# emanuele-artioli/elvis

Hardware: AMD Instinct MI355X
Metric: restored 1080p frames/sec, SinSR 4x path (ELVIS v2 Downsample) (higher is better)
Workload: dtype f16; 1 GPU; 30-frame 1920x1080 synthetic clip per GPU, ELVIS v2 Downsample (SinSR 4x), block 8, levels 0-3, weights seed 0 (random init), quantize=True; frames_per_gpu=30, parallelism=single GPU, gn_fused_into_conv=True, frames_per_invocation=15

## Files before the change

elvis_amd/_build.py:

```python
from __future__ import annotations

import os
import shutil
import subprocess
import sys
from concurrent.futures import ThreadPoolExecutor

HERE = os.path.dirname(os.path.abspath(__file__))
CSRC = os.path.join(HERE, "csrc")
LIBDIR = os.path.join(HERE, "lib")
OBJDIR = os.path.join(LIBDIR, "obj")
LIBPATH = os.path.join(LIBDIR, "libelvis_amd.so")
SOURCES = ["conv.hip", "conv_f32.hip", "dcn.hip", "swin.hip", "api.hip", "glue.hip", "misc.hip", "norm.hip", "attn.hip", "degrade.hip", "presley_degrade.hip", "classical.hip", "shrink.hip", "quality.hip", "handoff.hip"]
ARCH = "gfx950"
FLAGS = ["-O3", "-std=c++17", "-fPIC", f"--offload-arch={ARCH}", "-Wno-unused-result",
         "-ffp-contract=off"]
EXTRA_FLAGS = {"dcn.hip": ["-mllvm", "-pragma-unroll-threshold=262144"]}


def _hipcc() -> str:
    for cand in (shutil.which("hipcc"), "/opt/rocm/bin/hipcc"):
        if cand and os.path.exists(cand):
            return cand
    raise RuntimeError("hipcc not found; libelvis_amd cannot be built")


def _stale(target: str, deps) -> bool:
    if not os.path.exists(target):
        return True
    t = os.path.getmtime(target)
    return any(os.path.getmtime(d) > t for d in deps)


def build(force: bool = False, verbose: bool = True) -> str:
    os.makedirs(OBJDIR, exist_ok=True)
    hipcc = _hipcc()
    headers = [os.path.join(CSRC, f) for f in os.listdir(CSRC) if f.endswith((".h", ".inc"))]
    headers.append(os.path.join(os.path.dirname(HERE), "include", "elvis_amd.h"))
    jobs = []
    for src in SOURCES:
        s = os.path.join(CSRC, src)
        o = os.path.join(OBJDIR, src.replace(".hip", ".o"))
        if force or _stale(o, [s] + headers):
            jobs.append((s, o))

    def compile_one(job):
# ... 25 lines not shown
```

elvis_amd/_lib.py:

```python
from __future__ import annotations

import ctypes as C
import os
import threading
from typing import Optional

HERE = os.path.dirname(os.path.abspath(__file__))
LIBPATH = os.environ.get("ELVIS_AMD_LIB") or os.path.join(HERE, "lib", "libelvis_amd.so")

F32, F16 = 0, 1
ROUND_CV2, ROUND_HALF_UP = 0, 1
SSIM_LUMA, SSIM_CHANNELS = 0, 1
SSIM_REFLECT, SSIM_VALID = 0, 1
SSIM_PAD_AUTO = -1

_lock = threading.Lock()
_lib: Optional[C.CDLL] = None

vp, i32, f32, i64, f64 = C.c_void_p, C.c_int, C.c_float, C.c_longlong, C.c_double


class ConvDesc(C.Structure):
    _fields_ = [(n, C.c_int) for n in (
        "dtype", "n", "h", "w", "cin", "cin_pitch", "cin2", "cin2_pitch", "cout", "cout_pitch",
# ... 11 lines not shown
    "elvis_tile_accumulate_f32": [vp, vp, vp, vp, vp, vp, i32, i32, i32, i32, i32, i32, i32, f32, vp],
    "elvis_tile_normalize_u8": [vp, vp, vp, i32, i32, i32, vp],
    "elvis_sse_u8": [vp, vp, vp, vp, vp, i32, i32, i32, i32, vp],
    "elvis_block_ssim_u8": [vp, vp, vp, vp, i32, i32, i32, i32, i32, vp],
    "elvis_mask_bbox_u8": [vp, vp, i32, i32, i32, vp],
    "elvis_apply_mask_u8": [vp, vp, vp, i32, i32, i32, i32, i32, vp],
    "elvis_ssim_workspace_bytes": [i32, i32, i32, i32],
    "elvis_ssim_mean_f64": [vp, vp, vp, vp, vp, vp, vp, i32, i32, i32, i32, i32, i32, f64, f64, f64, i32, f64, vp],
    "elvis_u8_to_float": [vp, vp, i32, i32, i32, i32, i32, f32, f32, i32, i32, vp],
    "elvis_float_to_u8": [vp, i32, vp, vp, i32, i32, i32, i32, f32, f32, i32, i32, vp],
    "elvis_conv_packed_weight_bytes": [C.POINTER(ConvDesc)],
    "elvis_conv_pack_weights": [C.POINTER(ConvDesc), vp, vp, vp],
    "elvis_conv2d": [C.POINTER(ConvDesc), vp, vp, vp, vp, vp, i32, vp, vp, vp, vp, vp],
    "elvis_conv_stats_tiles": [C.POINTER(ConvDesc)],
    "elvis_conv_kernel_name": [C.POINTER(ConvDesc), C.c_char_p, C.c_size_t],
    "elvis_conv_kernel_name_for_call": [C.POINTER(ConvDesc), i32, i32, C.c_char_p, C.c_size_t],
    "elvis_conv_x3_eligible": [C.POINTER(ConvDesc)],
    "elvis_conv_debug_set": [C.c_char_p, i32],
    "elvis_gn_partials_to_sums": [vp, i32, i32, i32, vp, i32, i32, vp],
    "elvis_groupnorm_workspace_floats": [i32, i32, i32, i32],
    "elvis_groupnorm_sums": [vp, i32, i32, i32, i32, i32, vp, i32, i32, vp, vp],
    "elvis_groupnorm_affine": [vp, vp, vp, vp, vp, vp, vp, i32, i32, i32, i32, f32, vp],
    "elvis_affine_act": [vp, vp, i32, i32, i32, i32, i32, i32, vp, vp, i32, vp],
    "elvis_layernorm": [vp, vp, i32, i64, i32, i32, i32, vp, vp, f32, vp],
    "elvis_swin_packed_bytes": [i32, i32, i32],
    "elvis_swin_pack_weights": [vp, vp, vp, i32, i32, i32, vp],
    "elvis_swin_mlp": [vp, vp, vp, vp, vp, vp, vp, i64, i32, i32, i32, i32, f32, vp],
    "elvis_swin_ln_linear": [vp, vp, vp, vp, vp, vp, i64, i32, i32, i32, i32, f32, vp],
    "elvis_swin_pack_proj_mlp": [vp, vp, vp, vp, i32, i32, vp],
    "elvis_swin_proj_mlp": [vp, vp, vp, vp, vp, vp, vp, vp, vp, i64, i32, i32, i32, i32, i32, f32, vp],
    "elvis_window_attention": [vp, vp, i32, i32, i32, i32, i32, i32, i32, i32, i32, i32, vp, f32, vp],
    "elvis_bicubic_upsample": [vp, vp, i32, i32, i32, i32, i32, i32, i32, i32, vp],
    "elvis_vq_nearest": [vp, vp, vp, i32, i64, i32, i32, i32, vp, i32, vp],
    "elvis_pad_reflect_axpy": [vp, vp, i32, i32, i32, i32, i32, i32, i32, i32, i32, i32, f32, vp, f32, vp],
    "elvis_crop_copy": [vp, vp, i32, i32, i32, i32, i32, i32, i32, i32, i32, vp],
    "elvis_convert_act": [vp, i32, vp, i32, i64, i32, vp],
    "elvis_degrade_downsample_u8": [vp, vp, vp, i32, i32, i32, i32, i32, i32, i32, vp],
    "elvis_degrade_gaussian_u8": [vp, vp, vp, i32, i32, i32, i32, i32, i32, i32, f32, f32, f32, vp],
    "elvis_degrade_dct_u8": [vp, vp, vp, vp, vp, i32, i32, i32, i32, i32, i32, i32, vp],
    "elvis_degrade_scale_u8": [vp, vp, vp, i32, i32, i32, i32, i32, i32, i32, vp, vp, vp, i32, vp],
    "elvis_degrade_gaussian_fx_u8": [vp, vp, vp, i32, i32, i32, i32, i32, i32, i32, i32, i32, i32, vp],
    "elvis_rgb_to_i420_u8": [vp, vp, i32, i32, i32, i32, vp],
    "elvis_classical_lanczos_u8": [vp, vp, vp, i32, i32, i32, i32, i32, i32, i32, vp, vp],
    "elvis_classical_unsharp_u8": [vp, vp, vp, i32, i32, i32, i32, i32, i32, i32, i32, vp, vp, i32, vp],
    "elvis_temporal_blend_u8": [vp, vp, i32, i64, f64, f64, vp],
    "elvis_block_gather_u8": [vp, vp, vp, vp, i32, i32, i32, i32, i32, i32, i32, i32, i32, vp],
    "elvis_shrink_select_topk": [vp, vp, vp, i32, i32, i32, i32, vp],
    "elvis_shrink_passes_plan": [i32, i32, i32, i32, vp, vp, vp, i32],
    "elvis_shrink_select_passes": [vp, vp, vp, vp, vp, vp, i32, i32, i32, i32, i32, i32, i32, vp],
    "elvis_stretch_index": [vp, vp, i32, i32, i32, i32, i32, i32, vp],
    "elvis_dcnv2": [vp, vp, vp, vp, vp, i32, i32, i32, i32, i32, i32, i32, i32, i32, i32, i32, i32, vp],
    "elvis_temporal_stack": [vp, vp, i32, i32, i32, i32, i32, i32, i32, i32, vp],
    "elvis_plane_merge": [vp, vp, vp, i32, i32, i32, i32, i32, i32, vp],
}


def lib() -> C.CDLL:
    global _lib
    if _lib is not None:
        return _lib
    with _lock:
        if _lib is not None:
            return _lib
        if not os.path.exists(LIBPATH):
            raise RuntimeError(
                f"libelvis_amd.so not found at {LIBPATH}. Build it with `python -m elvis_amd._build` "
# ... 67 lines not shown
```

elvis_amd/csrc/norm.hip:

```cpp
#include "common.h"

namespace {

template <typename T> struct Vec16 {
    uint4 raw;
    __device__ __forceinline__ float get(int i) const { return to_f(reinterpret_cast<const T*>(&raw)[i]); }
    __device__ __forceinline__ void set(int i, float v) { reinterpret_cast<T*>(&raw)[i] = from_f<T>(v); }
};

template <typename T>
__global__ __launch_bounds__(256) void gn_channel_sums_kernel(const T* __restrict__ x, int hw, int c, int pitch,
                                                              int px_per_block, float* __restrict__ partials) {
    constexpr int VEC = DT<T>::VEC;
    extern __shared__ float red[];
    const int cv = (c + VEC - 1) / VEC;
    const int pl_count = 256 / cv;
    const int tid = threadIdx.x;
    const int vec = tid % cv, plane = tid / cv;
    const int n = blockIdx.y;
    const long long p0 = (long long)blockIdx.x * px_per_block;
    long long p1 = p0 + px_per_block;
    if (p1 > hw) p1 = hw;
    float s[VEC], ss[VEC];
#pragma unroll
// ... 32 lines not shown
    }
}

__global__ __launch_bounds__(256) void gn_partials_reduce_kernel(const float* __restrict__ partials,
                                                                 int tiles_per_image, int c,
                                                                 double* __restrict__ sums, int ctot, int coff) {
    __shared__ double ra[256], rb[256];
    const int ch = blockIdx.x, n = blockIdx.y, tid = threadIdx.x;
    double a = 0, b = 0;
    const float* base = partials + ((long long)n * tiles_per_image * c + ch) * 2;
    for (int t = tid; t < tiles_per_image; t += 256) {
        a += (double)base[(long long)t * c * 2 + 0];
        b += (double)base[(long long)t * c * 2 + 1];
    }
    ra[tid] = a;
    rb[tid] = b;
    __syncthreads();
    for (int o = 128; o > 0; o >>= 1) {
        if (tid < o) {
            ra[tid] += ra[tid + o];
            rb[tid] += rb[tid + o];
        }
        __syncthreads();
    }
    if (tid == 0) {
        sums[((long long)n * ctot + coff + ch) * 2 + 0] = ra[0];
        sums[((long long)n * ctot + coff + ch) * 2 + 1] = rb[0];
    }
}

__global__ __launch_bounds__(256) void gn_partials_reduce4_kernel(const float* __restrict__ partials,
                                                                  int tiles_per_image, int c,
                                                                  double* __restrict__ sums, int ctot, int coff) {
    __shared__ double red[8][256];
    const int ch = blockIdx.x * 4, n = blockIdx.y, tid = threadIdx.x;
    double acc[8] = {0, 0, 0, 0, 0, 0, 0, 0};
    const float* base = partials + ((long long)n * tiles_per_image * c + ch) * 2;
    for (int t = tid; t < tiles_per_image; t += 256) {
        const float4* p4 = reinterpret_cast<const float4*>(base + (long long)t * c * 2);
        const float4 u = p4[0], v = p4[1];
        acc[0] += (double)u.x; acc[1] += (double)u.y; acc[2] += (double)u.z; acc[3] += (double)u.w;
        acc[4] += (double)v.x; acc[5] += (double)v.y; acc[6] += (double)v.z; acc[7] += (double)v.w;
    }
#pragma unroll
    for (int k = 0; k < 8; ++k) red[k][tid] = acc[k];
    __syncthreads();
    for (int o = 128; o > 0; o >>= 1) {
        if (tid < o) {
#pragma unroll
            for (int k = 0; k < 8; ++k) red[k][tid] += red[k][tid + o];
        }
        __syncthreads();
    }
    if (tid < 8) sums[((long long)n * ctot + coff + ch) * 2 + tid] = red[tid][0];
}

__global__ void gn_affine_kernel(const double* __restrict__ sums, const float* __restrict__ gamma,
                                 const float* __restrict__ beta, const float* __restrict__ scale,
                                 const float* __restrict__ shift, float* __restrict__ pa, float* __restrict__ pb,
                                 int n, int hw, int c, int groups, float eps) {
    int i = blockIdx.x * blockDim.x + threadIdx.x;
    if (i >= n * c) return;
    int ni = i / c, ch = i - ni * c;
    int cpg = c / groups;
    int g = ch / cpg;
    double s = 0, ss = 0;
    for (int k = 0; k < cpg; ++k) {
        s += sums[((long long)ni * c + g * cpg + k) * 2 + 0];
        ss += sums[((long long)ni * c + g * cpg + k) * 2 + 1];
    }
    double cnt = (double)hw * cpg;
    double mean = s / cnt;
    double var = ss / cnt - mean * mean;
    if (var < 0) var = 0;
    float rstd = (float)(1.0 / sqrt(var + (double)eps));
    float ga = gamma ? gamma[ch] : 1.f, be = beta ? beta[ch] : 0.f;
    float a = rstd * ga;
    float b = be - (float)mean * a;
    if (scale) {
        float sc = 1.f + scale[ch];
        a *= sc;
        b = b * sc + (shift ? shift[ch] : 0.f);
    } else if (shift) {
        b += shift[ch];
    }
    pa[i] = a;
    pb[i] = b;
// ... 97 lines not shown
    ELVIS_REQUIRE(n > 0 && hw > 0 && c > 0 && pitch >= c && pitch % 8 == 0, "elvis_groupnorm_sums: bad shape c=%d pitch=%d", c, pitch);
    int vec = dtype == ELVIS_F16 ? 8 : 4;
    int cv = (c + vec - 1) / vec;
    ELVIS_REQUIRE(cv <= 256, "elvis_groupnorm_sums: too many channels (%d)", c);
    ELVIS_REQUIRE(sums_coff >= 0 && sums_coff + c <= sums_ctot, "elvis_groupnorm_sums: channel slice [%d,%d) outside %d", sums_coff, sums_coff + c, sums_ctot);
    ELVIS_REQUIRE((uintptr_t)x % 16 == 0, "elvis_groupnorm_sums: x must be 16-byte aligned");
    int pl = 256 / cv;
    int px_per_block = 0;
    int gx = gn_blocks(dtype, hw, c, &px_per_block);
    size_t lds = (size_t)pl * c * 2 * sizeof(float);
    ELVIS_REQUIRE(lds <= 64 * 1024, "elvis_groupnorm_sums: LDS budget exceeded");
    if (dtype == ELVIS_F16)
        hipLaunchKernelGGL(gn_channel_sums_kernel<half_t>, dim3(gx, n), dim3(256), lds, (hipStream_t)stream,
                           (const half_t*)x, hw, c, pitch, px_per_block, workspace);
    else if (dtype == ELVIS_F32)
        hipLaunchKernelGGL(gn_channel_sums_kernel<float>, dim3(gx, n), dim3(256), lds, (hipStream_t)stream,
                           (const float*)x, hw, c, pitch, px_per_block, workspace);
    else
        ELVIS_REQUIRE(false, "elvis_groupnorm_sums: bad dtype");
    ELVIS_CHECK_LAUNCH("elvis_groupnorm_sums");
    elvis_note_launch(dtype == ELVIS_F16 ? "gn_channel_sums_kernel<half>" : "gn_channel_sums_kernel<float>");
    hipLaunchKernelGGL(gn_partials_reduce_kernel, dim3(c, n), dim3(256), 0, (hipStream_t)stream, workspace, gx, c, sums,
                       sums_ctot, sums_coff);
    ELVIS_CHECK_LAUNCH("elvis_groupnorm_sums(reduce)");
    return ELVIS_OK;
}

extern "C" int elvis_gn_partials_to_sums(const float* partials, int tiles_per_image, int n, int c, double* sums,
                                         int sums_ctot, int sums_coff, elvis_stream_t stream) {
    ELVIS_REQUIRE(partials && sums && tiles_per_image > 0 && n > 0 && c > 0, "elvis_gn_partials_to_sums: bad argument");
    ELVIS_REQUIRE(sums_coff >= 0 && sums_coff + c <= sums_ctot, "elvis_gn_partials_to_sums: channel slice outside buffer");
    const bool four = c % 4 == 0 && ((uintptr_t)partials & 15) == 0;
    if (four)
        hipLaunchKernelGGL(gn_partials_reduce4_kernel, dim3(c / 4, n), dim3(256), 0, (hipStream_t)stream, partials,
                           tiles_per_image, c, sums, sums_ctot, sums_coff);
    else
        hipLaunchKernelGGL(gn_partials_reduce_kernel, dim3(c, n), dim3(256), 0, (hipStream_t)stream, partials,
                           tiles_per_image, c, sums, sums_ctot, sums_coff);
    ELVIS_CHECK_LAUNCH("elvis_gn_partials_to_sums");
    elvis_note_launch(four ? "gn_partials_reduce4_kernel" : "gn_partials_reduce_kernel");
    return ELVIS_OK;
}

extern "C" int elvis_groupnorm_affine(const double* sums, const float* gamma, const float* beta, const float* scale,
                                      const float* shift, float* pa, float* pb, int n, int hw, int c, int groups,
                                      float eps, elvis_stream_t stream) {
    ELVIS_REQUIRE(sums && pa && pb, "elvis_groupnorm_affine: null pointer");
    ELVIS_REQUIRE(n > 0 && hw > 0 && c > 0 && groups > 0 && c % groups == 0, "elvis_groupnorm_affine: c=%d not divisible by groups=%d", c, groups);
    int total = n * c;
    hipLaunchKernelGGL(gn_affine_kernel, dim3((total + 255) / 256), dim3(256), 0, (hipStream_t)stream, sums, gamma,
                       beta, scale, shift, pa, pb, n, hw, c, groups, eps);
    ELVIS_CHECK_LAUNCH("elvis_groupnorm_affine");
    elvis_note_launch("gn_affine_kernel");
    return ELVIS_OK;
}

extern "C" int elvis_affine_act(const void* x, void* y, int dtype, int n, int hw, int c, int pitch_in, int pitch_out,
                                const float* pa, const float* pb, int act, elvis_stream_t stream) {
    ELVIS_REQUIRE(x && y && pa && pb, "elvis_affine_act: null pointer");
    ELVIS_REQUIRE(n > 0 && hw > 0 && c > 0 && pitch_in >= c && pitch_out >= c && pitch_in % 8 == 0 && pitch_out % 8 == 0,
                  "elvis_affine_act: bad shape");
    ELVIS_REQUIRE(act == 0 || act == 2, "elvis_affine_act: act must be 0 or 2");
    ELVIS_REQUIRE(((uintptr_t)x | (uintptr_t)y) % 16 == 0, "elvis_affine_act: x and y must be 16-byte aligned");
    int vec = dtype == ELVIS_F16 ? 8 : 4;
    long long total_vec = (long long)n * hw * ((c + 7) / 8 * (8 / vec));
    int grid = (int)((total_vec + 255) / 256);
    if (grid > 256 * 32) grid = 256 * 32;
// ... 40 lines not shown
```

elvis_amd/ops.py:

```python
from __future__ import annotations

import ctypes as C
from dataclasses import dataclass
from typing import Optional

import numpy as np
import torch

from . import _lib as L
from ._lib import ConvDesc, check, lib, ptr


def _s(t: torch.Tensor) -> int:
    return torch.cuda.current_stream(t.device).cuda_stream


def pitch_for(c: int) -> int:
    return (c + 7) // 8 * 8


@dataclass
class Act:
    t: torch.Tensor
    c: int
# ... 517 lines not shown
        self.gamma, self.beta = norm_w.to(**f32).contiguous(), norm_b.to(**f32).contiguous()

    def __call__(self, x: Act, y: Optional[Act] = None) -> Act:
        if x.c != self.c or x.t.dtype != torch.float16:
            raise ValueError(f"fused Swin block: expected f16 with {self.c} channels, got {x.t.dtype} with {x.c}")
        if self.proj != (y is not None) or (y is not None and (y.c != self.c or y.t.dtype != torch.float16 or y.t.shape[:3] != x.t.shape[:3])):
            raise ValueError("fused Swin block: the projection form takes (attention output, residual stream) of one shape")
        tokens = x.n * x.h * x.w
        cout = self.c if self.mlp else self.n1
        out = new_act(x.n, x.h, x.w, cout, torch.float16, x.t.device, zero=False)
        if self.proj:
            with _Timed("swin_proj_mlp", "mfma", (4.0 * self.c * self.n1 + 2.0 * self.c * self.c) * tokens):
                check(lib().elvis_swin_proj_mlp(ptr(x.t), ptr(y.t), ptr(out.t), ptr(self.packed), ptr(self.bp), ptr(self.b1), ptr(self.b2),
                                                ptr(self.gamma), ptr(self.beta), tokens, self.c, self.n1, x.pitch, y.pitch, out.pitch,
                                                self.eps, _s(x.t)), x.t.device)
        elif self.mlp:
            with _Timed("swin_mlp", "mfma", 4.0 * self.c * self.n1 * tokens):
                check(lib().elvis_swin_mlp(ptr(x.t), ptr(out.t), ptr(self.packed), ptr(self.b1), ptr(self.b2), ptr(self.gamma),
                                           ptr(self.beta), tokens, self.c, self.n1, x.pitch, out.pitch, self.eps, _s(x.t)), x.t.device)
        else:
            with _Timed("swin_ln_linear", "hbm", 2.0 * (self.c + self.n1) * tokens):
                check(lib().elvis_swin_ln_linear(ptr(x.t), ptr(out.t), ptr(self.packed), ptr(self.b1), ptr(self.gamma), ptr(self.beta),
                                                 tokens, self.c, self.n1, x.pitch, out.pitch, self.eps, _s(x.t)), x.t.device)
        return out


def bicubic_upsample(x: Act, sf: int) -> Act:
    out = new_act(x.n, x.h * sf, x.w * sf, x.c, x.t.dtype, x.t.device, zero=False)
    check(lib().elvis_bicubic_upsample(ptr(x.t), ptr(out.t), x.dtype_code, x.n, x.h, x.w, x.c, x.pitch, out.pitch, sf,
                                       _s(x.t)), x.t.device)
    return out


def vq_nearest(z: Act, codebook: torch.Tensor, want_idx=False):
    out = new_act(z.n, z.h, z.w, z.c, z.t.dtype, z.t.device, zero=False)
    idx = torch.empty((z.n, z.h, z.w), dtype=torch.int32, device=z.t.device) if want_idx else None
    check(lib().elvis_vq_nearest(ptr(z.t), ptr(out.t), ptr(idx), z.dtype_code, z.n * z.h * z.w, z.c, z.pitch,
                                 out.pitch, ptr(codebook), codebook.shape[0], _s(z.t)), z.t.device)
    return (out, idx) if want_idx else out


def pad_reflect_axpy(x: Act, hp, wp, out: Act, ch_offset=0, mul=1.0, add=None, add_mul=0.0):
    check(lib().elvis_pad_reflect_axpy(ptr(x.t), ptr(out.t), x.dtype_code, x.n, x.h, x.w, x.c, x.pitch, hp, wp,
                                       out.pitch, ch_offset, float(mul), ptr(add), float(add_mul), _s(x.t)),
          x.t.device)
    return out


def crop_copy(x: Act, h, w) -> Act:
    out = new_act(x.n, h, w, x.c, x.t.dtype, x.t.device, zero=False)
    check(lib().elvis_crop_copy(ptr(x.t), ptr(out.t), x.dtype_code, x.n, x.h, x.w, x.pitch, h, w, x.c, out.pitch,
                                _s(x.t)), x.t.device)
    return out


def convert_act(x: Act, dtype) -> Act:
    if x.t.dtype == dtype:
        return x
    out = torch.empty(x.t.shape, dtype=dtype, device=x.t.device)
    check(lib().elvis_convert_act(ptr(x.t), x.dtype_code, ptr(out), L.dtype_code(dtype), x.n * x.h * x.w, x.pitch,
                                  _s(x.t)), x.t.device)
    return Act(out, x.c, x.stats if dtype == torch.float32 else None)


def dcnv2(x: Act, om: Act, weight: torch.Tensor, bias: Optional[torch.Tensor], groups: int, cout: int,
          mask_sigmoid: bool = True, act: int = 0) -> Act:
    out = new_act(x.n, x.h, x.w, cout, x.t.dtype, x.t.device)
    es = x.t.element_size()
    px_bytes = (27 * groups + x.c + cout) * es
    with _Timed("dcnv2", "hbm", float(px_bytes) * x.n * x.h * x.w):
        check(lib().elvis_dcnv2(ptr(x.t), ptr(om.t), ptr(weight), ptr(bias), ptr(out.t), x.dtype_code, x.n, x.h, x.w, x.c,
# ... 25 lines not shown
```

elvis_amd/sinsr.py:

```python
from __future__ import annotations

import math
from typing import Dict, List, Optional

import torch

from . import ops
from .ops import Act, PackedConv, PackedUpConv
from .weights import SinSRConfig, frame_noise, make_sinsr_weights, timestep_embedding, unet_layout


class _GN:
    def __init__(self, sd, p, device):
        self.gamma = sd[p + ".weight"].to(device=device, dtype=torch.float32).contiguous()
        self.beta = sd[p + ".bias"].to(device=device, dtype=torch.float32).contiguous()


def _conv(sd, p, dtype, device, cin, cin2=0) -> PackedConv:
    return PackedConv(sd[p + ".weight"], sd[p + ".bias"], dtype, device, cin, cin2)


class _DownConv:

    def __init__(self, sd, p, dtype, device, cin):
# ... 101 lines not shown

    SECTIONS = ("enc0", "enc1", "enc2", "unet", "dec2", "dec1", "dec0")
    MIXED_F16_DEFAULT = ("dec0",)
    DEC_SECTIONS = ("dec2", "dec1", "dec0")

    def __init__(self, cfg: SinSRConfig = SinSRConfig(), state_dict: Optional[Dict[str, torch.Tensor]] = None,
                 device="cuda:0", dtype=torch.float16, weight_seed: int = 0, fuse_gn: bool = True,
                 precision: Optional[str] = None):
        self.cfg, self.device, self.dtype, self.fuse_gn = cfg, torch.device(device), dtype, fuse_gn
        self.precision = precision or ("f16" if dtype == torch.float16 else "f32")
        if precision == "dec_f16":
            precision = "mixed:" + "+".join(self.DEC_SECTIONS)
        self.sec_dtype = {sec: dtype for sec in self.SECTIONS}
        self.x3 = precision is not None and (precision == "x3" or (precision.startswith("mixed") and not precision.startswith("mixed_exact")))
        if precision == "x3":
            self.dtype = dtype = torch.float32
            self.sec_dtype = {sec: dtype for sec in self.SECTIONS}
            precision = "f32"
        if precision is not None and precision.startswith("mixed"):
            f16 = tuple(precision.split(":", 1)[1].split("+")) if ":" in precision else self.MIXED_F16_DEFAULT
            unknown = [sec for sec in f16 if sec not in self.SECTIONS]
            if unknown:
                raise ValueError(f"unknown section(s) {unknown}; sections are {self.SECTIONS}")
            self.sec_dtype = {sec: (torch.float16 if sec in f16 else torch.float32) for sec in self.SECTIONS}
            self.dtype = self.sec_dtype["unet"]
        elif precision not in (None, "f16", "f32"):
            raise ValueError(f"unknown precision '{precision}'")
        sd = state_dict if state_dict is not None else make_sinsr_weights(cfg, weight_seed)
        dev = self.device
        with torch.cuda.device(dev), ops.x3_default(self.x3):
            self._build_unet(sd)
            self._build_ae(sd)
        self.codebook = sd["ae.quantize.embedding.weight"].to(device=dev, dtype=torch.float32).contiguous()

    def _build_unet(self, sd):
        cfg, dev, dt = self.cfg, self.device, self.sec_dtype["unet"]
        te0 = _linear(sd, "model.time_embed.0", torch.float32, dev)
        te2 = _linear(sd, "model.time_embed.2", torch.float32, dev)
        e = timestep_embedding(cfg.steps - 1, cfg.model_channels).to(dev)
        e = Act(e.view(1, 1, 1, -1).contiguous(), cfg.model_channels)
        e = te2(te0(e, act=2))
        ones = torch.ones((1, e.c), device=dev)
        zeros = torch.zeros((1, e.c), device=dev)
        silu_e = ops.affine_act(e, ones, zeros, act=2)
        plan = unet_layout(cfg)
        self.plan = plan

        def make(kind, p, meta, cin2=0):
            p = "model." + p
            if kind == "conv_in":
                return _conv(sd, p, dt, dev, meta[0])
            if kind == "res":
                cin, cout = meta[0] - cin2, meta[1]
                emb = _linear(sd, p + ".emb_layers.1", torch.float32, dev)(silu_e)
                ss = emb.t.view(-1)[: 2 * cout].clone()
                names = (p + ".in_layers.0", p + ".in_layers.2", p + ".out_layers.0", p + ".out_layers.3",
                         p + ".skip_connection")
                return _ResBlock(sd, names, cin, cin2, cout, dt, dev, cfg.gn_groups, 1e-5,
                                 scale=ss[:cout].contiguous(), shift=ss[cout:].contiguous())
            if kind == "swin":
                return _SwinLayer(sd, p, meta[0], cfg, dt, dev)
            if kind == "up":
                return _upconv(sd, p, dt, dev, meta[0])
            if kind == "down":
                return _conv(sd, p, dt, dev, meta[0])
            raise ValueError(kind)
# ... 78 lines not shown
                    h = m(h, stride=2)
                elif kind == "up":
                    h = m(h, want_stats=self.fuse_gn)
                else:
                    h = m(h)
            return h

        hs: List[Act] = []
        h = x
        for mods in self.u_input:
            h = run(mods, h)
            hs.append(h)
        h = run(self.u_middle, h)
        for mods in self.u_output:
            h = run(mods, h, hs.pop())
        return self._gn_silu_conv(h, self.u_out_norm, self.u_out_conv, 1e-5)

    def encode(self, x: Act) -> Act:
        h = self.e_conv_in(ops.convert_act(x, self.sec_dtype["enc0"]), want_stats=self.fuse_gn)
        for blocks, ds, dt in self.e_down:
            h = ops.convert_act(h, dt)
            for b in blocks:
                h = b(h, fuse_gn=self.fuse_gn)
            if ds is not None:
                h = ds(h, want_stats=self.fuse_gn)
        for b in self.e_mid:
            h = b(h, fuse_gn=self.fuse_gn)
        h = self._gn_silu_conv(h, self.e_norm_out, self.e_conv_out, 1e-6)
        return self.quant_conv(h)

    def decode(self, z: Act, quantize: Optional[bool] = None, want_idx=False):
        idx = None
        if self.cfg.quantize if quantize is None else quantize:
            z, idx = ops.vq_nearest(z, self.codebook, want_idx=True)
        z = ops.convert_act(z, self.sec_dtype[self._ae_section("dec", len(self.cfg.ae_ch_mult) - 1)])
        h = self.d_conv_in(self.post_quant_conv(z), want_stats=self.fuse_gn)
        for b in self.d_mid:
            h = b(h, fuse_gn=self.fuse_gn)
        for blocks, us, dt in self.d_up:
            h = ops.convert_act(h, dt)
            for b in blocks:
                h = b(h, fuse_gn=self.fuse_gn)
            if us is not None:
                h = us(h, want_stats=self.fuse_gn)
        out = self._gn_silu_conv(h, self.d_norm_out, self.d_conv_out, 1e-6)
        return (out, idx) if want_idx else out

    def padded_latent_shape(self, h, w):
        a = self.cfg.unet_align
        return (math.ceil(h / a) * a, math.ceil(w / a) * a)

    def forward(self, lr_u8: torch.Tensor, noise: torch.Tensor, *, swap_rb=False, want_f32=False,
                stages: Optional[dict] = None):
        cfg = self.cfg
        n, h, w, _ = lr_u8.shape
        hp, wp = self.padded_latent_shape(h, w)
        if tuple(noise.shape) != (n, cfg.latent_ch, hp, wp):
            raise ValueError(f"noise must be {(n, cfg.latent_ch, hp, wp)}, got {tuple(noise.shape)}")
        y = ops.u8_to_float(lr_u8, self.dtype, 2.0, -1.0, swap_rb=swap_rb, div255=True)
        y_up = ops.bicubic_upsample(ops.convert_act(y, self.sec_dtype["enc0"]), cfg.sf)
        z_y = ops.convert_act(self.encode(y_up), self.dtype)
        if stages is not None:
            stages["y_up"], stages["z_y"] = y_up, z_y
        del y_up
        std = math.sqrt(cfg.etas_end * cfg.kappa ** 2 + 1.0)
        uin = ops.new_act(n, hp, wp, 2 * cfg.latent_ch, self.dtype, self.device, zero=True)
        ops.pad_reflect_axpy(z_y, hp, wp, uin, 0, mul=1.0 / std, add=noise.contiguous(),
# ... 17 lines not shown
```

include/elvis_amd.h:

```cpp
#ifndef ELVIS_AMD_H
#define ELVIS_AMD_H

#include <stddef.h>
#include <stdint.h>

#ifdef __cplusplus
extern "C" {
#endif

#define ELVIS_ABI_VERSION 1

#define ELVIS_OK 0
#define ELVIS_E_INVALID (-1)
#define ELVIS_E_RUNTIME (-2)
#define ELVIS_E_UNSUPPORTED (-3)

#define ELVIS_F32 0
#define ELVIS_F16 1
#define ELVIS_F32X3 2

#define ELVIS_ROUND_CV2 0
#define ELVIS_ROUND_HALF_UP 1

typedef void* elvis_stream_t;
// ... 104 lines not shown
                           float eps, elvis_stream_t stream);


int elvis_affine_act(const void* x, void* y, int dtype, int n, int hw, int c, int pitch_in,
                     int pitch_out, const float* pa, const float* pb, int act, elvis_stream_t stream);

int elvis_layernorm(const void* x, void* y, int dtype, long long tokens, int c, int pitch_in,
                    int pitch_out, const float* gamma, const float* beta, float eps, elvis_stream_t stream);

size_t elvis_swin_packed_bytes(int c, int n1, int mode);
int elvis_swin_pack_weights(const float* w1, const float* w2, void* packed, int c, int n1, int mlp, elvis_stream_t stream);
int elvis_swin_mlp(const void* x, void* out, const void* packed, const float* b1, const float* b2, const float* gamma,
                   const float* beta, long long tokens, int c, int hidden, int x_pitch, int out_pitch, float eps,
                   elvis_stream_t stream);
int elvis_swin_ln_linear(const void* x, void* out, const void* packed, const float* bias, const float* gamma, const float* beta,
                         long long tokens, int c, int n_out, int x_pitch, int out_pitch, float eps, elvis_stream_t stream);
int elvis_swin_pack_proj_mlp(const float* wp, const float* w1, const float* w2, void* packed, int c, int hidden, elvis_stream_t stream);
int elvis_swin_proj_mlp(const void* attn, const void* y, void* out, const void* packed, const float* bp, const float* b1,
                        const float* b2, const float* gamma, const float* beta, long long tokens, int c, int hidden,
                        int attn_pitch, int y_pitch, int out_pitch, float eps, elvis_stream_t stream);

const char* elvis_last_launch(void);

int elvis_window_attention(const void* qkv, void* out, int dtype, int n, int h, int w, int heads,
                           int head_dim, int ws, int shift, int qkv_pitch, int out_pitch,
                           const float* bias_table, float scale, elvis_stream_t stream);

int elvis_bicubic_upsample(const void* x, void* y, int dtype, int n, int h, int w, int c, int pitch_in,
                           int pitch_out, int sf, elvis_stream_t stream);

int elvis_vq_nearest(const void* z, void* zq, int32_t* idx_out, int dtype, long long pixels, int c,
                     int pitch_in, int pitch_out, const float* codebook, int n_embed, elvis_stream_t stream);

int elvis_pad_reflect_axpy(const void* x, void* y, int dtype, int n, int h, int w, int c, int pitch_in,
                           int hp, int wp, int pitch_out, int ch_offset_out, float mul, const float* add,
                           float add_mul, elvis_stream_t stream);

int elvis_crop_copy(const void* x, void* y, int dtype, int n, int h_in, int w_in, int pitch_in, int h,
                    int w, int c, int pitch_out, elvis_stream_t stream);

int elvis_convert_act(const void* x, int src_dtype, void* y, int dst_dtype, long long pixels, int pitch,
                      elvis_stream_t stream);


int elvis_degrade_downsample_u8(const uint8_t* src, const int32_t* levels, uint8_t* dst, int n, int h, int w, int c,
                                int block_size, int by, int bx, elvis_stream_t stream);

int elvis_degrade_gaussian_u8(const uint8_t* src, const int32_t* rounds, uint8_t* dst, int n, int h, int w, int c,
                              int block_size, int by, int bx, float tap0, float tap1, float tap2, elvis_stream_t stream);

int elvis_degrade_dct_u8(const uint8_t* src, const int32_t* levels, uint8_t* dst, const float* basis64, const float* gain,
                         int n_levels, int n, int h, int w, int c, int by, int bx, elvis_stream_t stream);


#define ELVIS_DEGRADE_MAX_ROUNDS 64

int elvis_degrade_scale_u8(const uint8_t* src, const int32_t* scales, uint8_t* dst, int n, int h, int w, int c,
                           int block_size, int by, int bx, const int32_t* tab_starts, const int32_t* tab_src,
                           const float* tab_w, int tab_len, elvis_stream_t stream);

int elvis_degrade_gaussian_fx_u8(const uint8_t* src, const int32_t* rounds, uint8_t* dst, int n, int h, int w, int c,
                                 int block_size, int by, int bx, int tap0, int tap1, int tap2, elvis_stream_t stream);


int elvis_rgb_to_i420_u8(const uint8_t* src, uint8_t* dst, int n, int h, int w, int bgr, elvis_stream_t stream);

// ... 50 lines not shown
```

Measured before the change: 31.21 frames/s.

## Add grid-bucketed spatial index for 3-D VQ nearest lookup; widen GN partial reduce

Builds a uniform 3-D grid index over the VQ codebook once at load time. Each cell stores the codes that could be nearest to any point in it, so the decode quantizer scans only the candidates for a pixel's cell instead of the whole codebook, and falls back to a wavefront-cooperative full scan for points outside the grid. Separately, the GroupNorm partials reduction now handles 16 channels per block instead of 4 with rotated shared-memory indexing, cutting the block count. The index costs extra memory and host-synchronous build work at init, and its exactness depends on the conservative cell bounds and tie-breaking matching the original kernel.

```diff
diff --git a/elvis_amd/_build.py b/elvis_amd/_build.py
--- a/elvis_amd/_build.py
+++ b/elvis_amd/_build.py
@@ -11,7 +11,7 @@
 LIBDIR = os.path.join(HERE, "lib")
 OBJDIR = os.path.join(LIBDIR, "obj")
 LIBPATH = os.path.join(LIBDIR, "libelvis_amd.so")
-SOURCES = ["conv.hip", "conv_f32.hip", "dcn.hip", "swin.hip", "api.hip", "glue.hip", "misc.hip", "norm.hip", "attn.hip", "degrade.hip", "presley_degrade.hip", "classical.hip", "shrink.hip", "quality.hip", "handoff.hip"]
+SOURCES = ["conv.hip", "conv_f32.hip", "dcn.hip", "swin.hip", "api.hip", "glue.hip", "misc.hip", "vq_index.hip", "norm.hip", "attn.hip", "degrade.hip", "presley_degrade.hip", "classical.hip", "shrink.hip", "quality.hip", "handoff.hip"]
 ARCH = "gfx950"
 FLAGS = ["-O3", "-std=c++17", "-fPIC", f"--offload-arch={ARCH}", "-Wno-unused-result",
          "-ffp-contract=off"]
diff --git a/elvis_amd/_lib.py b/elvis_amd/_lib.py
--- a/elvis_amd/_lib.py
+++ b/elvis_amd/_lib.py
@@ -67,6 +67,9 @@
     "elvis_window_attention": [vp, vp, i32, i32, i32, i32, i32, i32, i32, i32, i32, i32, vp, f32, vp],
     "elvis_bicubic_upsample": [vp, vp, i32, i32, i32, i32, i32, i32, i32, i32, vp],
     "elvis_vq_nearest": [vp, vp, vp, i32, i64, i32, i32, i32, vp, i32, vp],
+    "elvis_vq_index_bytes": [vp, i32, i32, C.POINTER(C.c_size_t), vp],
+    "elvis_vq_index_build": [vp, i32, i32, vp, C.c_size_t, vp],
+    "elvis_vq_nearest_indexed": [vp, vp, vp, i32, i64, i32, i32, i32, vp, i32, vp, C.c_size_t, vp],
     "elvis_pad_reflect_axpy": [vp, vp, i32, i32, i32, i32, i32, i32, i32, i32, i32, i32, f32, vp, f32, vp],
     "elvis_crop_copy": [vp, vp, i32, i32, i32, i32, i32, i32, i32, i32, i32, vp],
     "elvis_convert_act": [vp, i32, vp, i32, i64, i32, vp],
diff --git a/elvis_amd/csrc/norm.hip b/elvis_amd/csrc/norm.hip
--- a/elvis_amd/csrc/norm.hip
+++ b/elvis_amd/csrc/norm.hip
@@ -88,27 +88,43 @@
 __global__ __launch_bounds__(256) void gn_partials_reduce4_kernel(const float* __restrict__ partials,
                                                                   int tiles_per_image, int c,
                                                                   double* __restrict__ sums, int ctot, int coff) {
-    __shared__ double red[8][256];
-    const int ch = blockIdx.x * 4, n = blockIdx.y, tid = threadIdx.x;
-    double acc[8] = {0, 0, 0, 0, 0, 0, 0, 0};
-    const float* base = partials + ((long long)n * tiles_per_image * c + ch) * 2;
-    for (int t = tid; t < tiles_per_image; t += 256) {
-        const float4* p4 = reinterpret_cast<const float4*>(base + (long long)t * c * 2);
-        const float4 u = p4[0], v = p4[1];
-        acc[0] += (double)u.x; acc[1] += (double)u.y; acc[2] += (double)u.z; acc[3] += (double)u.w;
-        acc[4] += (double)v.x; acc[5] += (double)v.y; acc[6] += (double)v.z; acc[7] += (double)v.w;
-    }
-#pragma unroll
-    for (int k = 0; k < 8; ++k) red[k][tid] = acc[k];
+    __shared__ double red[32][256];
+    const int ch = blockIdx.x * 16, n = blockIdx.y, tid = threadIdx.x;
+    const int q = tid & 7, r = tid >> 3;
+    const int nk = (c - ch < 16 ? c - ch : 16) * 2;
+    const bool live = q * 4 < nk;
+    double acc[8][4];
+#pragma unroll
+    for (int m = 0; m < 8; ++m)
+#pragma unroll
+        for (int i = 0; i < 4; ++i) acc[m][i] = 0;
+    const float* base = partials + ((long long)n * tiles_per_image * c + ch) * 2 + q * 4;
+    if (live) {
+        for (int t0 = 0; t0 < tiles_per_image; t0 += 256) {
+#pragma unroll
+            for (int m = 0; m < 8; ++m) {
+                const int t = t0 + m * 32 + r;
+                if (t < tiles_per_image) {
+                    const float4 u = *reinterpret_cast<const float4*>(base + (long long)t * c * 2);
+                    acc[m][0] += (double)u.x; acc[m][1] += (double)u.y; acc[m][2] += (double)u.z; acc[m][3] += (double)u.w;
+                }
+            }
+        }
+#pragma unroll
+        for (int m = 0; m < 8; ++m)
+#pragma unroll
+            for (int i = 0; i < 4; ++i) red[q * 4 + i][(m * 32 + r + 8 * q) & 255] = acc[m][i];
+    }
     __syncthreads();
-    for (int o = 128; o > 0; o >>= 1) {
-        if (tid < o) {
-#pragma unroll
-            for (int k = 0; k < 8; ++k) red[k][tid] += red[k][tid + o];
+    for (int sh = 7; sh >= 0; --sh) {
+        const int o = 1 << sh;
+        for (int i = tid; i < nk * o; i += 256) {
+            const int k = i >> sh, t = i & (o - 1), rot = 8 * (k >> 2);
+            red[k][(t + rot) & 255] += red[k][(t + o + rot) & 255];
         }
         __syncthreads();
     }
-    if (tid < 8) sums[((long long)n * ctot + coff + ch) * 2 + tid] = red[tid][0];
+    if (tid < nk) sums[((long long)n * ctot + coff + ch) * 2 + tid] = red[tid][(8 * (tid >> 2)) & 255];
 }
 
 __global__ void gn_affine_kernel(const double* __restrict__ sums, const float* __restrict__ gamma,
@@ -272,7 +288,7 @@
     ELVIS_REQUIRE(sums_coff >= 0 && sums_coff + c <= sums_ctot, "elvis_gn_partials_to_sums: channel slice outside buffer");
     const bool four = c % 4 == 0 && ((uintptr_t)partials & 15) == 0;
     if (four)
-        hipLaunchKernelGGL(gn_partials_reduce4_kernel, dim3(c / 4, n), dim3(256), 0, (hipStream_t)stream, partials,
+        hipLaunchKernelGGL(gn_partials_reduce4_kernel, dim3((c + 15) / 16, n), dim3(256), 0, (hipStream_t)stream, partials,
                            tiles_per_image, c, sums, sums_ctot, sums_coff);
     else
         hipLaunchKernelGGL(gn_partials_reduce_kernel, dim3(c, n), dim3(256), 0, (hipStream_t)stream, partials,
diff --git a/elvis_amd/csrc/vq_index.hip b/elvis_amd/csrc/vq_index.hip
--- /dev/null
+++ b/elvis_amd/csrc/vq_index.hip
@@ -0,0 +1,324 @@
+#include "common.h"
+#include <vector>
+#include <math.h>
+#include <string.h>
+
+namespace {
+
+constexpr int VQH_INTS = 16;
+constexpr int VQ_MAGIC = 0x56514958;
+constexpr int VQ_MAX_G = 16;
+constexpr float VQ_BEST0 = 3.0e38f;
+constexpr int VQ_NONE = 0x7fffffff;
+
+int vq_grid_side(int n_embed) {
+    int g = 1;
+    while (g < VQ_MAX_G && (long long)(g + 1) * (g + 1) * (g + 1) * 2 <= n_embed) ++g;
+    return g;
+}
+size_t vq_off_ints(int g) { return (size_t)(((long long)g * g * g + 1 + 3) / 4 * 4); }
+size_t vq_head_bytes(int g) { return (VQH_INTS + vq_off_ints(g)) * 4; }
+
+struct VqGrid {
+    int g;
+    float lo[3], inv[3];
+    double lo_d[3], h[3], eps[3];
+};
+
+__global__ __launch_bounds__(64) void vq_index_build_kernel(const float* __restrict__ codebook, int n_embed, VqGrid gr,
+                                                            int fill, int* __restrict__ counts,
+                                                            const int* __restrict__ off, float4* __restrict__ entries) {
+    const int cell = blockIdx.x, lane = threadIdx.x, g = gr.g;
+    const int cx = cell % g, cy = (cell / g) % g, cz = cell / (g * g);
+    const int cc[3] = {cx, cy, cz};
+    double a[3], b[3];
+#pragma unroll
+    for (int d = 0; d < 3; ++d) {
+        a[d] = gr.lo_d[d] + (double)cc[d] * gr.h[d] - gr.eps[d];
+        b[d] = gr.lo_d[d] + (double)(cc[d] + 1) * gr.h[d] + gr.eps[d];
+    }
+    double u = INFINITY;
+    for (int k = lane; k < n_embed; k += 64) {
+        double s = 0;
+#pragma unroll
+        for (int d = 0; d < 3; ++d) {
+            const double x = (double)codebook[(long long)k * 3 + d];
+            const double m = fmax(fabs(x - a[d]), fabs(x - b[d]));
+            s += m * m;
+        }
+        u = fmin(u, s);
+    }
+#pragma unroll
+    for (int o = 32; o > 0; o >>= 1) u = fmin(u, __shfl_xor(u, o, 64));
+    const double thr = u * (1.0 + 0x1p-18) + 1e-36;
+    int run = 0;
+    const int base0 = fill ? off[cell] : 0;
+    for (int base = 0; base < n_embed; base += 64) {
+        const int k = base + lane;
+        bool keep = false;
+        float x[3] = {0.f, 0.f, 0.f};
+        if (k < n_embed) {
+            double s = 0;
+#pragma unroll
+            for (int d = 0; d < 3; ++d) {
+                x[d] = codebook[(long long)k * 3 + d];
+                const double xd = (double)x[d];
+                const double m = fmax(fmax(a[d] - xd, xd - b[d]), 0.0);
+                s += m * m;
+            }
+            keep = s <= thr;
+        }
+        const unsigned long long mask = __ballot(keep);
+        if (fill && keep) {
+            const int pos = __popcll(mask & ((1ull << lane) - 1ull));
+            entries[base0 + run + pos] = make_float4(x[0], x[1], x[2], __int_as_float(k));
+        }
+        run += __popcll(mask);
+    }
+    if (!fill && lane == 0) counts[cell] = run;
+}
+
+__device__ __forceinline__ float vq_dist3(float z0, float z1, float z2, float c0, float c1, float c2) {
+    const float d0 = __fsub_rn(z0, c0), d1 = __fsub_rn(z1, c1), d2 = __fsub_rn(z2, c2);
+    return __fadd_rn(__fadd_rn(__fmul_rn(d0, d0), __fmul_rn(d1, d1)), __fmul_rn(d2, d2));
+}
+
+template <typename T>
+__global__ __launch_bounds__(256) void vq_cell_scan_kernel(const T* __restrict__ z, T* __restrict__ zq,
+                                                           int32_t* __restrict__ idx_out, long long pixels,
+                                                           int pitch_in, int pitch_out,
+                                                           const float* __restrict__ codebook, int n_embed, int g,
+                                                           const int* __restrict__ index) {
+    const long long px = (long long)blockIdx.x * blockDim.x + threadIdx.x;
+    const int lane = threadIdx.x & 63;
+    const bool active = px < pixels;
+    const float* hf = reinterpret_cast<const float*>(index);
+    const int* off = index + VQH_INTS;
+    const float4* entries = reinterpret_cast<const float4*>(index + VQH_INTS + (((long long)g * g * g + 1 + 3) / 4) * 4);
+    float zv[3] = {0.f, 0.f, 0.f};
+    if (active) {
+#pragma unroll
+        for (int k = 0; k < 3; ++k) zv[k] = to_f(z[px * pitch_in + k]);
+    }
+    const float gf = (float)g;
+    float t[3];
+#pragma unroll
+    for (int k = 0; k < 3; ++k) t[k] = __fmul_rn(__fsub_rn(zv[k], hf[4 + k]), hf[7 + k]);
+    const bool inside = active && t[0] >= 0.f && t[0] < gf && t[1] >= 0.f && t[1] < gf && t[2] >= 0.f && t[2] < gf;
+    float best = VQ_BEST0;
+    int best_i = VQ_NONE;
+    if (inside) {
+        const int cell = ((int)t[2] * g + (int)t[1]) * g + (int)t[0];
+        const int e0 = off[cell], e1 = off[cell + 1];
+        for (int e = e0; e < e1; ++e) {
+            const float4 en = entries[e];
+            const float d = vq_dist3(zv[0], zv[1], zv[2], en.x, en.y, en.z);
+            if (d < best) {
+                best = d;
+                best_i = __float_as_int(en.w);
+            }
+        }
+    }
+    unsigned long long todo = __ballot(active && !inside);
+    while (todo) {
+        const int src = __ffsll((long long)todo) - 1;
+        todo &= todo - 1;
+        const float s0 = __shfl(zv[0], src, 64), s1 = __shfl(zv[1], src, 64), s2 = __shfl(zv[2], src, 64);
+        float lb = VQ_BEST0;
+        int li = VQ_NONE;
+        for (int k = lane; k < n_embed; k += 64) {
+            const float d = vq_dist3(s0, s1, s2, codebook[(long long)k * 3], codebook[(long long)k * 3 + 1],
+                                     codebook[(long long)k * 3 + 2]);
+            if (d < lb) {
+                lb = d;
+                li = k;
+            }
+        }
+#pragma unroll
+        for (int o = 1; o < 64; o <<= 1) {
+            const float od = __shfl_xor(lb, o, 64);
+            const int oi = __shfl_xor(li, o, 64);
+            if (od < lb || (od == lb && oi < li)) {
+                lb = od;
+                li = oi;
+            }
+        }
+        if (lane == src) {
+            best = lb;
+            best_i = li;
+        }
+    }
+    if (active) {
+        if (idx_out) idx_out[px] = best_i;
+        const bool none = best_i == VQ_NONE;
+#pragma unroll
+        for (int k = 0; k < 3; ++k)
+            zq[px * pitch_out + k] = from_f<T>(none ? 0.f : codebook[(long long)best_i * 3 + k]);
+        for (int k = 3; k < pitch_out; ++k) zq[px * pitch_out + k] = from_f<T>(0.f);
+    }
+}
+
+bool vq_plan(const std::vector<float>& cb, int n_embed, VqGrid* gr) {
+    const int g = vq_grid_side(n_embed);
+    gr->g = g;
+    for (int d = 0; d < 3; ++d) {
+        double mn = INFINITY, mx = -INFINITY;
+        for (int k = 0; k < n_embed; ++k) {
+            const double v = (double)cb[(size_t)k * 3 + d];
+            if (!(fabs(v) <= 1e15)) {
+                elvis_set_error("elvis_vq_index: code %d is not finite or beyond 1e15", k);
+                return false;
+            }
+            mn = fmin(mn, v);
+            mx = fmax(mx, v);
+        }
+        const double margin = 0.25 * (mx - mn) + fmax(1e-3 * fmax(fabs(mn), fabs(mx)), 1e-6);
+        const float lo = (float)(mn - margin);
+        const float inv = (float)((double)g / ((mx + margin) - (double)lo));
+        gr->lo[d] = lo;
+        gr->inv[d] = inv;
+        gr->lo_d[d] = (double)lo;
+        gr->h[d] = 1.0 / (double)inv;
+        gr->eps[d] = 0x1p-21 * (double)g * gr->h[d];
+    }
+    return true;
+}
+
+int vq_fetch_codebook(const float* codebook, int n_embed, hipStream_t s, std::vector<float>* host, const char* who) {
+    host->resize((size_t)n_embed * 3);
+    hipError_t e = hipMemcpyAsync(host->data(), codebook, host->size() * 4, hipMemcpyDeviceToHost, s);
+    if (e == hipSuccess) e = hipStreamSynchronize(s);
+    if (e != hipSuccess) {
+        elvis_set_error("%s: reading the codebook failed: %s", who, hipGetErrorString(e));
+        return ELVIS_E_RUNTIME;
+    }
+    return ELVIS_OK;
+}
+
+int vq_count(const float* codebook, int n_embed, const VqGrid& gr, int* counts_dev, hipStream_t s,
+             std::vector<int>* counts, const char* who) {
+    const int cells = gr.g * gr.g * gr.g;
+    hipLaunchKernelGGL(vq_index_build_kernel, dim3(cells), dim3(64), 0, s, codebook, n_embed, gr, 0, counts_dev,
+                       (const int*)nullptr, (float4*)nullptr);
+    ELVIS_CHECK_LAUNCH(who);
+    counts->resize(cells);
+    hipError_t e = hipMemcpyAsync(counts->data(), counts_dev, (size_t)cells * 4, hipMemcpyDeviceToHost, s);
+    if (e == hipSuccess) e = hipStreamSynchronize(s);
+    if (e != hipSuccess) {
+        elvis_set_error("%s: counting failed: %s", who, hipGetErrorString(e));
+        return ELVIS_E_RUNTIME;
+    }
+    return ELVIS_OK;
+}
+
+}
+
+extern "C" int elvis_vq_index_bytes(const float* codebook, int n_embed, int c, size_t* bytes_out,
+                                    elvis_stream_t stream) {
+    const char* who = "elvis_vq_index_bytes";
+    ELVIS_REQUIRE(codebook && bytes_out, "%s: null pointer", who);
+    ELVIS_REQUIRE(c == 3, "%s: the index takes 3-dimensional codebooks only (c = %d)", who, c);
+    ELVIS_REQUIRE(n_embed > 0 && n_embed <= (1 << 24), "%s: n_embed %d out of range", who, n_embed);
+    hipStream_t s = (hipStream_t)stream;
+    std::vector<float> host;
+    int rc = vq_fetch_codebook(codebook, n_embed, s, &host, who);
+    if (rc != ELVIS_OK) return rc;
+    VqGrid gr;
+    if (!vq_plan(host, n_embed, &gr)) return ELVIS_E_INVALID;
+    const int cells = gr.g * gr.g * gr.g;
+    int* counts_dev = nullptr;
+    hipError_t e = hipMalloc(&counts_dev, (size_t)cells * 4);
+    if (e != hipSuccess) {
+        elvis_set_error("%s: %s", who, hipGetErrorString(e));
+        return ELVIS_E_RUNTIME;
+    }
+    std::vector<int> counts;
+    rc = vq_count(codebook, n_embed, gr, counts_dev, s, &counts, who);
+    (void)hipFree(counts_dev);
+    if (rc != ELVIS_OK) return rc;
+    size_t total = 0;
+    for (int v : counts) total += (size_t)v;
+    *bytes_out = vq_head_bytes(gr.g) + total * 16;
+    return ELVIS_OK;
+}
+
+extern "C" int elvis_vq_index_build(const float* codebook, int n_embed, int c, void* index, size_t index_bytes,
+                                    elvis_stream_t stream) {
+    const char* who = "elvis_vq_index_build";
+    ELVIS_REQUIRE(codebook && index, "%s: null pointer", who);
+    ELVIS_REQUIRE(c == 3, "%s: the index takes 3-dimensional codebooks only (c = %d)", who, c);
+    ELVIS_REQUIRE(n_embed > 0 && n_embed <= (1 << 24), "%s: n_embed %d out of range", who, n_embed);
+    ELVIS_REQUIRE(((uintptr_t)index & 15) == 0, "%s: the index must be 16-byte aligned", who);
+    const int g0 = vq_grid_side(n_embed);
+    ELVIS_REQUIRE(index_bytes >= vq_head_bytes(g0), "%s: %zu bytes are less than the index header (%zu)", who, index_bytes,
+                  vq_head_bytes(g0));
+    hipStream_t s = (hipStream_t)stream;
+    std::vector<float> host;
+    int rc = vq_fetch_codebook(codebook, n_embed, s, &host, who);
+    if (rc != ELVIS_OK) return rc;
+    VqGrid gr;
+    if (!vq_plan(host, n_embed, &gr)) return ELVIS_E_INVALID;
+    const int cells = gr.g * gr.g * gr.g;
+    int* words = (int*)index;
+    std::vector<int> counts;
+    rc = vq_count(codebook, n_embed, gr, words + VQH_INTS, s, &counts, who);
+    if (rc != ELVIS_OK) return rc;
+    std::vector<int> head(VQH_INTS + vq_off_ints(gr.g), 0);
+    long long total = 0;
+    for (int cidx = 0; cidx < cells; ++cidx) {
+        head[VQH_INTS + cidx] = (int)total;
+        total += counts[cidx];
+    }
+    head[VQH_INTS + cells] = (int)total;
+    ELVIS_REQUIRE(total < (1ll << 31) && vq_head_bytes(gr.g) + (size_t)total * 16 <= index_bytes,
+                  "%s: the index needs %zu bytes, the buffer has %zu", who, vq_head_bytes(gr.g) + (size_t)total * 16, index_bytes);
+    head[0] = VQ_MAGIC;
+    head[1] = gr.g;
+    head[2] = n_embed;
+    head[3] = (int)total;
+    for (int d = 0; d < 3; ++d) {
+        memcpy(&head[4 + d], &gr.lo[d], 4);
+        memcpy(&head[7 + d], &gr.inv[d], 4);
+    }
+    hipError_t e = hipMemcpyAsync(words, head.data(), head.size() * 4, hipMemcpyHostToDevice, s);
+    if (e != hipSuccess) {
+        elvis_set_error("%s: writing the header failed: %s", who, hipGetErrorString(e));
+        return ELVIS_E_RUNTIME;
+    }
+    hipLaunchKernelGGL(vq_index_build_kernel, dim3(cells), dim3(64), 0, s, codebook, n_embed, gr, 1, (int*)nullptr,
+                       (const int*)(words + VQH_INTS), (float4*)(words + VQH_INTS + vq_off_ints(gr.g)));
+    ELVIS_CHECK_LAUNCH(who);
+    e = hipStreamSynchronize(s);
+    if (e != hipSuccess) {
+        elvis_set_error("%s: %s", who, hipGetErrorString(e));
+        return ELVIS_E_RUNTIME;
+    }
+    elvis_note_launch("vq_index_build_kernel");
+    return ELVIS_OK;
+}
+
+extern "C" int elvis_vq_nearest_indexed(const void* z, void* zq, int32_t* idx_out, int dtype, long long pixels, int c,
+                                        int pitch_in, int pitch_out, const float* codebook, int n_embed,
+                                        const void* index, size_t index_bytes, elvis_stream_t stream) {
+    const char* who = "elvis_vq_nearest_indexed";
+    ELVIS_REQUIRE(z && zq && codebook && index && pixels > 0, "%s: bad argument", who);
+    ELVIS_REQUIRE(n_embed > 0 && n_embed <= (1 << 24), "%s: n_embed %d out of range", who, n_embed);
+    ELVIS_REQUIRE(c == 3, "%s: c must be 3 (elvis_vq_nearest takes the others)", who);
+    ELVIS_REQUIRE(pitch_in >= c && pitch_out >= c, "%s: bad pitch", who);
+    ELVIS_REQUIRE(dtype == ELVIS_F16 || dtype == ELVIS_F32, "%s: bad dtype", who);
+    ELVIS_REQUIRE(((uintptr_t)index & 15) == 0, "%s: the index must be 16-byte aligned", who);
+    const int g = vq_grid_side(n_embed);
+    ELVIS_REQUIRE(index_bytes >= vq_head_bytes(g), "%s: %zu bytes are less than the index header (%zu)", who, index_bytes,
+                  vq_head_bytes(g));
+    ELVIS_REQUIRE((pixels + 255) / 256 <= 0x7fffffffll, "%s: too many pixels", who);
+    const int grid = (int)((pixels + 255) / 256);
+    if (dtype == ELVIS_F16)
+        hipLaunchKernelGGL(vq_cell_scan_kernel<half_t>, dim3(grid), dim3(256), 0, (hipStream_t)stream, (const half_t*)z,
+                           (half_t*)zq, idx_out, pixels, pitch_in, pitch_out, codebook, n_embed, g, (const int*)index);
+    else
+        hipLaunchKernelGGL(vq_cell_scan_kernel<float>, dim3(grid), dim3(256), 0, (hipStream_t)stream, (const float*)z,
+                           (float*)zq, idx_out, pixels, pitch_in, pitch_out, codebook, n_embed, g, (const int*)index);
+    ELVIS_CHECK_LAUNCH(who);
+    elvis_note_launch(dtype == ELVIS_F16 ? "vq_cell_scan_kernel<half>" : "vq_cell_scan_kernel<float>");
+    return ELVIS_OK;
+}
diff --git a/elvis_amd/ops.py b/elvis_amd/ops.py
--- a/elvis_amd/ops.py
+++ b/elvis_amd/ops.py
@@ -573,11 +573,32 @@
     return out
 
 
-def vq_nearest(z: Act, codebook: torch.Tensor, want_idx=False):
+VQ_INDEX_MAX_BYTES = 64 << 20
+
+
+def vq_index_build(codebook: torch.Tensor, max_bytes: int = VQ_INDEX_MAX_BYTES) -> Optional[torch.Tensor]:
+    if codebook.dim() != 2 or codebook.shape[1] != 3 or codebook.dtype != torch.float32 or not codebook.is_contiguous():
+        raise ValueError("vq_index_build: the codebook must be a contiguous [n_embed, 3] float32 tensor")
+    nbytes = C.c_size_t(0)
+    with torch.cuda.device(codebook.device):
+        check(lib().elvis_vq_index_bytes(ptr(codebook), codebook.shape[0], 3, C.byref(nbytes), _s(codebook)), codebook.device)
+        if nbytes.value > max_bytes:
+            return None
+        index = torch.empty(nbytes.value, dtype=torch.uint8, device=codebook.device)
+        check(lib().elvis_vq_index_build(ptr(codebook), codebook.shape[0], 3, ptr(index), nbytes.value, _s(codebook)), codebook.device)
+    return index
+
+
+def vq_nearest(z: Act, codebook: torch.Tensor, want_idx=False, index: Optional[torch.Tensor] = None):
     out = new_act(z.n, z.h, z.w, z.c, z.t.dtype, z.t.device, zero=False)
     idx = torch.empty((z.n, z.h, z.w), dtype=torch.int32, device=z.t.device) if want_idx else None
-    check(lib().elvis_vq_nearest(ptr(z.t), ptr(out.t), ptr(idx), z.dtype_code, z.n * z.h * z.w, z.c, z.pitch,
-                                 out.pitch, ptr(codebook), codebook.shape[0], _s(z.t)), z.t.device)
+    if index is not None and z.c == 3:
+        check(lib().elvis_vq_nearest_indexed(ptr(z.t), ptr(out.t), ptr(idx), z.dtype_code, z.n * z.h * z.w, z.c, z.pitch,
+                                             out.pitch, ptr(codebook), codebook.shape[0], ptr(index), index.numel(),
+                                             _s(z.t)), z.t.device)
+    else:
+        check(lib().elvis_vq_nearest(ptr(z.t), ptr(out.t), ptr(idx), z.dtype_code, z.n * z.h * z.w, z.c, z.pitch,
+                                     out.pitch, ptr(codebook), codebook.shape[0], _s(z.t)), z.t.device)
     return (out, idx) if want_idx else out
 
 
diff --git a/elvis_amd/sinsr.py b/elvis_amd/sinsr.py
--- a/elvis_amd/sinsr.py
+++ b/elvis_amd/sinsr.py
@@ -157,6 +157,7 @@
             self._build_unet(sd)
             self._build_ae(sd)
         self.codebook = sd["ae.quantize.embedding.weight"].to(device=dev, dtype=torch.float32).contiguous()
+        self.vq_index = ops.vq_index_build(self.codebook) if self.codebook.shape[1] == 3 else None
 
     def _build_unet(self, sd):
         cfg, dev, dt = self.cfg, self.device, self.sec_dtype["unet"]
@@ -301,7 +302,7 @@
     def decode(self, z: Act, quantize: Optional[bool] = None, want_idx=False):
         idx = None
         if self.cfg.quantize if quantize is None else quantize:
-            z, idx = ops.vq_nearest(z, self.codebook, want_idx=True)
+            z, idx = ops.vq_nearest(z, self.codebook, want_idx=True, index=self.vq_index)
         z = ops.convert_act(z, self.sec_dtype[self._ae_section("dec", len(self.cfg.ae_ch_mult) - 1)])
         h = self.d_conv_in(self.post_quant_conv(z), want_stats=self.fuse_gn)
         for b in self.d_mid:
diff --git a/include/elvis_amd.h b/include/elvis_amd.h
--- a/include/elvis_amd.h
+++ b/include/elvis_amd.h
@@ -160,6 +160,12 @@
 int elvis_vq_nearest(const void* z, void* zq, int32_t* idx_out, int dtype, long long pixels, int c,
                      int pitch_in, int pitch_out, const float* codebook, int n_embed, elvis_stream_t stream);
 
+int elvis_vq_index_bytes(const float* codebook, int n_embed, int c, size_t* bytes_out, elvis_stream_t stream);
+int elvis_vq_index_build(const float* codebook, int n_embed, int c, void* index, size_t index_bytes, elvis_stream_t stream);
+int elvis_vq_nearest_indexed(const void* z, void* zq, int32_t* idx_out, int dtype, long long pixels, int c,
+                             int pitch_in, int pitch_out, const float* codebook, int n_embed, const void* index,
+                             size_t index_bytes, elvis_stream_t stream);
+
 int elvis_pad_reflect_axpy(const void* x, void* y, int dtype, int n, int h, int w, int c, int pitch_in,
                            int hp, int wp, int pitch_out, int ch_offset_out, float mul, const float* add,
                            float add_mul, elvis_stream_t stream);
```

Measured after the change: 31.51 frames/s, median of 6. No clear change (+1.0%).
